# dkaslovsky/GraphRole

Measured on AMD Instinct MI355X. Metric: ReFeX edges-aggregated/sec (+ RolX NMF iters/sec in nmf.iters_per_s), 1M-node graph, higher is better.
Workload: dtype f64; 1 GPU; ba1m; description=Barabasi-Albert n=1,000,000 m=10 (~10M edges), seed 0  [BASELINE config 3/4], n_nodes=1000000, n_edges=9999900, nnz=19999800, n_roles=6, n_features=20

## Files before the change

### graphrole_amd/csrc/grx_common.h

```cpp
#pragma once
#include <hip/hip_runtime.h>

#include <cstdint>
#include <cstdio>

#include "grx.h"

void grx_set_error(const char *fmt, ...);

#define GRX_CHECK_HIP(expr)                                                                   \
    do {                                                                                      \
        hipError_t e__ = (expr);                                                              \
        if (e__ != hipSuccess) {                                                              \
            grx_set_error("%s:%d: %s -> %s", __FILE__, __LINE__, #expr, hipGetErrorString(e__)); \
            return GRX_ERR_HIP;                                                               \
        }                                                                                     \
    } while (0)

#define GRX_REQUIRE(cond, ...)                                                                \
    do {                                                                                      \
        if (!(cond)) {                                                                        \
            grx_set_error(__VA_ARGS__);                                                       \
            return GRX_ERR_INVALID;                                                           \
        }                                                                                     \
// ... 37 lines not shown
static inline size_t grx_align_up(size_t x, size_t a) { return (x + a - 1) / a * a; }

static inline unsigned grx_grid(int64_t items, int64_t per_block, int64_t cap)
{
    const int64_t g = grx_ceil_div(items, per_block);
    return (unsigned)(g < 1 ? 1 : g > cap ? cap : g);
}

void grx_fill32(int32_t *d_dst, int64_t count, int32_t value, hipStream_t st);
void grx_fill64(uint64_t *d_dst, int64_t count, uint64_t value, hipStream_t st);

struct SpPull {
    int64_t n;
    const int64_t *row_ptr;
    const int32_t *col;
    const double *w;
    const int32_t *hub_rows;
    int64_t n_hub_rows, hub_degree;
};

enum { GRX_CT_DONE = 0, GRX_CT_LEVEL, GRX_CT_FOUND, GRX_CT_BFS_WORDS };
constexpr int GRX_CTRL_MAX_WORDS = 16;

int grx_read_ctrl(const int32_t *d_ctrl, int words, int32_t *out, hipStream_t st);

int grx_frontier_advance(int32_t *d_ctrl, hipStream_t st);

template <class Enqueue>
int grx_run_rounds(const char *what, int batch, int64_t max_rounds, int words, const int32_t *d_ctrl, int32_t *h,
                   hipStream_t st, Enqueue enqueue_one)
{
    for (int k = 0; k < words; ++k) h[k] = 0;
    int64_t issued = 0;
    while (!h[0]) {
        GRX_REQUIRE(issued <= max_rounds, what, (long long)issued);
        for (int k = 0; k < batch; ++k, ++issued) {
            const int rc = enqueue_one();
            if (rc != GRX_OK) return rc;
            GRX_LAUNCH_CHECK();
        }
        const int rc = grx_read_ctrl(d_ctrl, words, h, st);
        if (rc != GRX_OK) return rc;
    }
    return GRX_OK;
}

int grx_internal_sort_columns(int64_t n, int ncols, const double *cols, int64_t ld, double *out, int64_t out_ld,
                              void *workspace, hipStream_t st);
int grx_internal_sort_pairs(int64_t n, const double *col, double *out, uint32_t *perm, void *workspace, hipStream_t st);
size_t grx_internal_sort_pairs_workspace_bytes(int64_t n);
int grx_internal_sort_u64(int64_t n, const uint64_t *keys, uint64_t *out, void *workspace, hipStream_t st);
int grx_internal_vertical_log_bin(int64_t n, int ncols, const double *d_cols, int64_t ld, const uint8_t *h_is_i64, double frac,
                                  uint8_t *d_bins, int64_t ld_bins, int32_t *d_nbins, void *d_workspace,
                                  size_t workspace_bytes, int32_t *d_status, void *stream);
int64_t grx_internal_plan_max_degree(const grx_aggregate_plan *plan);

#ifndef GRX_NT_STREAMS
#define GRX_NT_STREAMS 0
#endif
#if GRX_NT_STREAMS
#define GRX_STREAM_LD(p) __builtin_nontemporal_load(&(p))
#define GRX_STREAM_ST(p, v) __builtin_nontemporal_store((v), &(p))
#else
#define GRX_STREAM_LD(p) (p)
#define GRX_STREAM_ST(p, v) ((p) = (v))
#endif

template <int WIDTH>
__device__ __forceinline__ double grx_group_sum(double v)
{
#pragma unroll
    for (int off = WIDTH / 2; off > 0; off >>= 1) v += __shfl_xor(v, off, WIDTH);
    return v;
}

template <int WIDTH>
__device__ __forceinline__ double grx_group_max(double v)
{
#pragma unroll
    for (int off = WIDTH / 2; off > 0; off >>= 1) v = fmax(v, __shfl_xor(v, off, WIDTH));
    return v;
}

template <int BLOCK, bool MAX = false>
__device__ __forceinline__ double grx_block_reduce(double v, double *sm)
{
    const int t = threadIdx.x;
    sm[t] = v;
    __syncthreads();
#pragma unroll
    for (int s = BLOCK / 2; s > 0; s >>= 1) {
        if (t < s) sm[t] = MAX ? fmax(sm[t], sm[t + s]) : sm[t] + sm[t + s];
        __syncthreads();
    }
    const double r = sm[0];
    __syncthreads();
    return r;
}
```

### graphrole_amd/csrc/grx_prune.hip

```cpp
#include "grx_sort.h"

#include <cstdlib>

namespace {

struct BinPlanCol {
    uint64_t const_bits;
    uint8_t narrow;
    uint8_t npass;
    uint8_t lo_shift;
    uint8_t pad0;
    uint8_t dshift[4];
};

struct ColFlags { uint64_t w[8]; };
constexpr int MAX_TYPED_COLS = 512;
__device__ __forceinline__ bool col_is_i64(const ColFlags &f, int col) { return col < MAX_TYPED_COLS && ((f.w[col >> 6] >> (col & 63)) & 1ull); }
__device__ __forceinline__ uint64_t i64_bits_to_key(double raw) { return (uint64_t)__double_as_longlong(raw) ^ 0x8000000000000000ull; }
__device__ __forceinline__ uint64_t value_key(double raw, bool is_i64) { return is_i64 ? i64_bits_to_key(raw) : f64_to_key(raw + 0.0); }

constexpr int BITS_TILE = 256 * 32;
constexpr int LO_SHIFT_INT = 255;

__global__ __launch_bounds__(256) void key_bits_kernel(const double *__restrict__ cols, int64_t ld, int64_t n,
// ... 688 lines not shown
                pq[u] = act[u] ? pair_pq[id] : 0u;
            }
            uint2 x[U], y[U];
#pragma unroll
            for (int u = 0; u < U; ++u) {
                act[u] = act[u] && (int)cur[u] <= cap;
                x[u] = *reinterpret_cast<const uint2 *>(tile + (pq[u] >> 8) * CH_STRIDE + lane * 8);
                y[u] = *reinterpret_cast<const uint2 *>(tile + (pq[u] & 0xFF) * CH_STRIDE + lane * 8);
            }
#pragma unroll
            for (int u = 0; u < U; ++u) {
                if (!act[u]) continue;
                const int id = id0 + 4 * u;
                uint32_t m = ch_absdiff_max4(x[u].x, y[u].x);
                const uint32_t m2 = ch_absdiff_max4(x[u].y, y[u].y);
                m = m2 > m ? m2 : m;
                if (__ballot((int)m > cap) != 0) {
                    if (lane == 0) pair_max[id] = (uint8_t)(cap + 1);
                    continue;
                }
#pragma unroll
                for (int off = 32; off > 0; off >>= 1) {
                    const uint32_t o = __shfl_xor(m, off, 64);
                    m = o > m ? o : m;
                }
                if (lane == 0 && m > cur[u]) pair_max[id] = (uint8_t)m;
            }
        }
    }
    __syncthreads();
    for (int id = threadIdx.x; id < npairs; id += 256) {
        const int mx = pair_max[id];
        if (mx == 0) continue;
        const int lp = pair_pq[id] >> 8, lq = pair_pq[id] & 0xFF;
        const int p = lp < na ? a0 + lp : b0 + (lp - na), q = lq < na ? a0 + lq : b0 + (lq - na);
        if (__hip_atomic_load(&dist[(size_t)p * ldF + q], __ATOMIC_RELAXED, __HIP_MEMORY_SCOPE_AGENT) < mx) {
            atomicMax(&dist[(size_t)p * ldF + q], mx);
            atomicMax(&dist[(size_t)q * ldF + p], mx);
        }
    }
}

constexpr int SEL_NB = 4096;
constexpr int SEL_MAX_IDS = 512;
constexpr int SEL_SORT_CAP = 8192;
constexpr uint16_t SEL_MARK_SORTED = 0x8000;
constexpr uint16_t SEL_MARK_TIES = 0xFFFF;
constexpr uint16_t SEL_THR_EXACT = 0x8000;
inline int64_t sel_bid_min_n()
{
    static const int64_t v = [] { const char *e = std::getenv("GRX_BIN_BID_MIN_N"); return e ? (int64_t)std::atoll(e) : (int64_t)2500000; }();
    return v;
}
__host__ __device__ inline int64_t sel_bid_stride(int64_t n) { return (n + 3) & ~(int64_t)3; }
constexpr int SEL_HIST_ITEMS = 32;
constexpr int SEL_HIST_TILE = 256 * SEL_HIST_ITEMS;
struct SelMap { uint64_t kmin; int shift; int ncells; int nb; };
constexpr int SEL_NSAMPLE = SEL_NB - 1;

__device__ __forceinline__ int sel_bucket(const SelMap &m, const uint32_t *__restrict__ lut, uint64_t key)
{
    if (key <= m.kmin) return 0;
    const uint64_t rel = key - m.kmin;
    uint64_t c = rel >> m.shift;
    if (c >= (uint64_t)m.ncells) return m.nb - 1;
    const uint32_t e = lut[c];
    const int k = (int)(e >> 16);
    const uint64_t within = rel - (c << m.shift);
    return (int)(e & 0xFFFFu) + (int)(within >> (m.shift - k));
}

constexpr int SEL_MAX_TIES = 511;

__global__ __launch_bounds__(1024) void sel_map_kernel(const double *__restrict__ cols, int64_t ld, int64_t n,
                                                       SelMap *__restrict__ maps, uint32_t *__restrict__ luts,
                                                       uint16_t *__restrict__ tie_of_bucket, uint64_t *__restrict__ tie_value,
                                                       uint32_t *__restrict__ hist, uint32_t *__restrict__ cursor,
                                                       unsigned long long *__restrict__ bmin,
                                                       unsigned long long *__restrict__ bmax, uint8_t *__restrict__ tie_broken,
                                                       int32_t *__restrict__ fault, ColFlags flags)
{
    for (int b = threadIdx.x; b < SEL_NB; b += 1024) {
        const size_t cell = (size_t)blockIdx.x * SEL_NB + b;
        hist[cell] = 0; cursor[cell] = 0; bmax[cell] = 0ull; bmin[cell] = ~0ull; tie_broken[cell] = 0;
    }
    if (blockIdx.x == 0 && threadIdx.x == 0) *fault = 0;
    __shared__ unsigned long long smin[SEL_NB];
    __shared__ unsigned long long smax[SEL_NB];
    __shared__ uint32_t scnt[SEL_NB];
    __shared__ uint32_t s_lut[SEL_NB];
    __shared__ uint32_t cnt[SEL_NB];
    __shared__ uint64_t red[32];
    __shared__ uint32_t wsum[16];
    __shared__ SelMap s_map;
    const int col = blockIdx.x, t = threadIdx.x, lane = t & 63, wave = t >> 6;
    const bool i64 = col_is_i64(flags, col);
    const double *x = cols + (size_t)col * ld;
    uint64_t key[4];
    bool have[4];
    uint64_t mn = ~0ull, mx = 0ull;
#pragma unroll
    for (int j = 0; j < 4; ++j) {
        const int64_t k = (int64_t)t * 4 + j;
        have[j] = k < SEL_NSAMPLE && (n > SEL_NSAMPLE || k < n);
        key[j] = 0;
        if (have[j]) {
            key[j] = value_key(x[n > SEL_NSAMPLE ? (k * (n - 1)) / (SEL_NSAMPLE - 1) : k], i64);
            mn = key[j] < mn ? key[j] : mn;
            mx = key[j] > mx ? key[j] : mx;
        }
        cnt[4 * t + j] = 0;
    }
#pragma unroll
    for (int off = 32; off > 0; off >>= 1) {
        const uint64_t a = __shfl_xor(mn, off, 64), b = __shfl_xor(mx, off, 64);
        mn = a < mn ? a : mn;
        mx = b > mx ? b : mx;
    }
    if (lane == 0) { red[wave] = mn; red[16 + wave] = mx; }
    __syncthreads();
    if (t == 0) {
        for (int w = 1; w < 16; ++w) { mn = red[w] < mn ? red[w] : mn; mx = red[16 + w] > mx ? red[16 + w] : mx; }
        const uint64_t span = mx - mn;
        const int bits = span ? 64 - __clzll((long long)span) : 0;
        s_map.kmin = mn;
        s_map.shift = bits > 12 ? bits - 12 : 0;
        s_map.ncells = (int)(span >> s_map.shift) + 1;
        s_map.nb = 0;
    }
    __syncthreads();
    const SelMap m = s_map;
#pragma unroll
    for (int j = 0; j < 4; ++j)
// ... 19 lines not shown
    __syncthreads();
    uint32_t run = inc - local;
    for (int w = 0; w < wave; ++w) run += wsum[w];
    uint32_t *lut = luts + (size_t)col * SEL_NB;
#pragma unroll
    for (int j = 0; j < 4; ++j) {
        const uint32_t e = run | (kk[j] << 16);
        lut[4 * t + j] = e;
        s_lut[4 * t + j] = e;
        run += alloc[j];
        smin[4 * t + j] = ~0ull; smax[4 * t + j] = 0ull; scnt[4 * t + j] = 0;
    }
    if (t == 1023) {
        s_map.nb = (int)run + 1;
        maps[col] = s_map;
    }
    __syncthreads();
    const SelMap mm = s_map;
#pragma unroll
    for (int j = 0; j < 4; ++j) {
        if (have[j]) {
            const int b = sel_bucket(mm, s_lut, key[j]);
            atomicAdd(&scnt[b], 1u);
            atomicMin(&smin[b], (unsigned long long)key[j]);
            atomicMax(&smax[b], (unsigned long long)key[j]);
        }
    }
    __syncthreads();
    uint32_t cand[4];
#pragma unroll
    for (int j = 0; j < 4; ++j) { const int b = 4 * t + j; cand[j] = (scnt[b] >= 2 && smin[b] == smax[b]) ? 1u : 0u; }
    const uint32_t lc = cand[0] + cand[1] + cand[2] + cand[3];
    uint32_t ic = lc;
#pragma unroll
    for (int off = 1; off < 64; off <<= 1) {
        const uint32_t y = __shfl_up(ic, off, 64);
        if (lane >= off) ic += y;
    }
    __syncthreads();
    if (lane == 63) wsum[wave] = ic;
    __syncthreads();
    uint32_t id = ic - lc;
    for (int w = 0; w < wave; ++w) id += wsum[w];
#pragma unroll
    for (int j = 0; j < 4; ++j) {
        const int b = 4 * t + j;
        uint16_t tid = 0;
        if (cand[j]) {
            ++id;
            if (id <= SEL_MAX_TIES) { tid = (uint16_t)id; tie_value[(size_t)col * (SEL_MAX_TIES + 1) + id] = smin[b]; }
        }
        tie_of_bucket[(size_t)col * SEL_NB + b] = tid;
    }
}

template <bool STORE_BID>
__global__ __launch_bounds__(256) void sel_hist_kernel(const double *__restrict__ cols, int64_t ld, int64_t n,
                                                       const SelMap *__restrict__ maps, const uint32_t *__restrict__ luts,
                                                       const uint16_t *__restrict__ tie_of_bucket,
                                                       const uint64_t *__restrict__ tie_value, uint8_t *__restrict__ tie_broken,
                                                       uint32_t *__restrict__ hist, uint16_t *__restrict__ bid, ColFlags flags,
                                                       int tiles_per_wg)
{
    __shared__ uint32_t h[SEL_NB];
    __shared__ uint32_t lut[SEL_NB];
    __shared__ uint16_t tieb[SEL_NB];
    __shared__ uint64_t tiev[SEL_MAX_TIES + 1];
    const int col = blockIdx.y;
    const bool i64 = col_is_i64(flags, col);
    const SelMap m = maps[col];
    for (int b = threadIdx.x; b < SEL_NB; b += 256) {
        h[b] = 0;
        lut[b] = luts[(size_t)col * SEL_NB + b];
        tieb[b] = tie_of_bucket[(size_t)col * SEL_NB + b];
    }
    for (int k = threadIdx.x; k <= SEL_MAX_TIES; k += 256) tiev[k] = tie_value[(size_t)col * (SEL_MAX_TIES + 1) + k];
    __syncthreads();
    const double *x = cols + (size_t)col * ld;
    const int64_t last = n - 1;
    const int lane = threadIdx.x & 63;
    for (int tile = 0; tile < tiles_per_wg; ++tile) {
    const int64_t base = ((int64_t)blockIdx.x * tiles_per_wg + tile) * SEL_HIST_TILE;
    if (base >= n) break;
    for (int i0 = 0; i0 < SEL_HIST_ITEMS; i0 += 8) {
        double raw[8];
#pragma unroll
        for (int j = 0; j < 8; ++j) {
            const int64_t idx = base + (int64_t)(i0 + j) * 256 + threadIdx.x;
            raw[j] = x[idx < n ? idx : last];
        }
        __builtin_amdgcn_sched_barrier(0);
#pragma unroll
        for (int j = 0; j < 8; ++j) {
            const bool valid = base + (int64_t)(i0 + j) * 256 + threadIdx.x < n;
            const uint64_t key = value_key(raw[j], i64);
            const int b = sel_bucket(m, lut, key);
            if (STORE_BID && valid)
                bid[(size_t)col * sel_bid_stride(n) + base + (int64_t)(i0 + j) * 256 + threadIdx.x] = (uint16_t)b;
            const int tid = valid ? (int)tieb[b] : 0;
            if (tid && tiev[tid] != key) tie_broken[(size_t)col * SEL_NB + b] = 1;
            const uint64_t active = __ballot(valid);
            if (active == 0) continue;
            const int b0 = __shfl(b, __ffsll((long long)active) - 1, 64);
            if (__ballot(valid && b != b0) == 0) {
                if (lane == __ffsll((long long)active) - 1) atomicAdd(&h[b0], (uint32_t)__popcll(active));
            } else if (valid) {
                atomicAdd(&h[b], 1u);
            }
        }
    }
    }
    __syncthreads();
    uint32_t *out = hist + (size_t)col * SEL_NB;
    for (int b = threadIdx.x; b < SEL_NB; b += 256)
        if (h[b]) atomicAdd(&out[b], h[b]);
}

__global__ __launch_bounds__(1024) void sel_walk1_kernel(int64_t n, double frac,
                                                         const uint32_t *__restrict__ hist, const uint16_t *__restrict__ tie_of_bucket,
                                                         const uint8_t *__restrict__ tie_broken,
                                                         const uint64_t *__restrict__ tie_value, uint32_t *__restrict__ cum,
                                                         uint16_t *__restrict__ mark, uint32_t *__restrict__ seg_off,
                                                         uint16_t *__restrict__ idlist, int32_t *__restrict__ nids,
                                                         unsigned long long *__restrict__ bmin,
                                                         unsigned long long *__restrict__ bmax)
{
    __shared__ uint8_t TIE[SEL_NB];
    __shared__ uint32_t C[SEL_NB];
    __shared__ uint32_t S[SEL_NB];
    __shared__ uint8_t M[SEL_NB];
    __shared__ uint32_t wsum[16];
    const int col = blockIdx.x, t = threadIdx.x, lane = t & 63, wave = t >> 6;
    constexpr int nb = SEL_NB;
    const uint32_t *h = hist + (size_t)col * SEL_NB;
    auto scan4 = [&](uint32_t (&v)[4], uint32_t *dst) {
        const uint32_t local = v[0] + v[1] + v[2] + v[3];
        uint32_t inc = local;
#pragma unroll
        for (int off = 1; off < 64; off <<= 1) {
            const uint32_t y = __shfl_up(inc, off, 64);
            if (lane >= off) inc += y;
        }
        __syncthreads();
        if (lane == 63) wsum[wave] = inc;
        __syncthreads();
        uint32_t before = inc - local;
        for (int w = 0; w < wave; ++w) before += wsum[w];
        uint32_t run = before;
#pragma unroll
        for (int j = 0; j < 4; ++j) { run += v[j]; dst[4 * t + j] = run; }
        __syncthreads();
    };
    uint32_t v[4];
#pragma unroll
    for (int j = 0; j < 4; ++j) {
        const int b = 4 * t + j;
        v[j] = b < nb ? h[b] : 0u;
        M[b] = 0;
        TIE[b] = (tie_of_bucket[(size_t)col * SEL_NB + b] != 0 && tie_broken[(size_t)col * SEL_NB + b] == 0) ? 1 : 0;
    }
    scan4(v, C);
    if (wave == 0) {
        auto bucket_of = [&](int64_t pos) {
            const int coarse = lane * 64 + 63;
            const bool gt = coarse < nb ? (int64_t)C[coarse] > pos : true;
            const int blk = __ffsll((long long)__ballot(gt)) - 1;
            const int fine = blk * 64 + lane;
            const bool gt2 = fine < nb ? (int64_t)C[fine] > pos : true;
            return blk * 64 + __ffsll((long long)__ballot(gt2)) - 1;
        };
        int64_t dlo = 0, dhi = 0;
        for (int step = 0; step < GRX_MAX_BINS && dlo < n; ++step) {
            int64_t slo = (int64_t)(frac * (double)(n - dlo));
            if (slo < 1) slo = 1;
            const int64_t plo = dlo + slo - 1;
            const int64_t dh = dhi < n ? dhi : n - 1;
            int64_t shi = (int64_t)(frac * (double)(n - dh));
            if (shi < 1) shi = 1;
            int64_t phi = dh + shi - 1;
            if (phi < plo) phi = plo;
            const int jlo = bucket_of(plo), jhi = bucket_of(phi);
            for (int j = jlo + lane; j <= jhi; j += 64) M[j] = 1;
            dlo = TIE[jlo] ? (int64_t)C[jlo] : plo + 1;
            dhi = (int64_t)C[jhi];
            if (dhi < dlo) dhi = dlo;
        }
    }
    __syncthreads();
    bool collect[4];
#pragma unroll
    for (int j = 0; j < 4; ++j) {
        const int b = 4 * t + j;
        const uint32_t cnt = b < nb ? (C[b] - (b ? C[b - 1] : 0u)) : 0u;
        collect[j] = M[b] && !TIE[b];
        v[j] = collect[j] ? cnt : 0u;
        if (M[b] && TIE[b]) {
            const size_t cell = (size_t)col * SEL_NB + b;
            const uint64_t value = tie_value[(size_t)col * (SEL_MAX_TIES + 1) + tie_of_bucket[cell]];
            bmin[cell] = value;
            bmax[cell] = value;
        }
    }
    scan4(v, S);
#pragma unroll
    for (int j = 0; j < 4; ++j) {
        const int b = 4 * t + j;
        if (b < nb) {
            cum[(size_t)col * SEL_NB + b] = C[b];
            seg_off[(size_t)col * SEL_NB + b] = S[b] - v[j];
        }
    }
    uint32_t m[4];
#pragma unroll
    for (int j = 0; j < 4; ++j) m[j] = collect[j] ? 1u : 0u;
    scan4(m, S);
#pragma unroll
    for (int j = 0; j < 4; ++j) {
        const int b = 4 * t + j;
        if (b < nb) {
            const uint32_t id = S[b];
            uint16_t mk = 0;
            if (m[j]) {
                mk = (uint16_t)(id < SEL_MAX_IDS ? id : SEL_MAX_IDS);
                if (id < SEL_MAX_IDS) idlist[(size_t)col * SEL_MAX_IDS + id - 1] = (uint16_t)b;
            } else if (M[b]) {
                mk = SEL_MARK_TIES;
            }
            mark[(size_t)col * SEL_NB + b] = mk;
        }
    }
    if (t == 1023) nids[col] = (int32_t)(S[nb - 1] < (uint32_t)SEL_MAX_IDS ? S[nb - 1] : SEL_MAX_IDS - 1);
}

__global__ __launch_bounds__(512) void sel_sort_kernel(const uint32_t *__restrict__ cum, const uint32_t *__restrict__ seg_off,
                                                       const uint16_t *__restrict__ idlist, const int32_t *__restrict__ nids,
                                                       const unsigned long long *__restrict__ bmin,
                                                       const unsigned long long *__restrict__ bmax, int64_t n,
                                                       uint64_t *__restrict__ coll, uint16_t *__restrict__ mark)
{
    __shared__ uint64_t s[SEL_SORT_CAP];
    const int col = blockIdx.y;
    const int count = nids[col];
    for (int id = blockIdx.x; id < count; id += gridDim.x) {
        const int b = idlist[(size_t)col * SEL_MAX_IDS + id];
        const size_t cell = (size_t)col * SEL_NB + b;
        const int64_t len = (int64_t)cum[cell] - (b ? (int64_t)cum[cell - 1] : 0);
        if (len < 2 || len > SEL_SORT_CAP || bmin[cell] == bmax[cell]) continue;
        uint64_t *seg = coll + (size_t)col * n + seg_off[cell];
        int P = 2;
        while (P < len) P <<= 1;
        __syncthreads();
        for (int i = threadIdx.x; i < P; i += 512) s[i] = i < len ? seg[i] : ~0ull;
        for (int k = 2; k <= P; k <<= 1) {
            for (int j = k >> 1; j > 0; j >>= 1) {
                __syncthreads();
                for (int i = threadIdx.x; i < P / 2; i += 512) {
                    const int lo = 2 * i - (i & (j - 1)), hi = lo + j;
                    const uint64_t a = s[lo], c = s[hi];
                    const bool up = (lo & k) == 0;
                    if ((a > c) == up) { s[lo] = c; s[hi] = a; }
                }
            }
        }
        __syncthreads();
        for (int i = threadIdx.x; i < len; i += 512) seg[i] = s[i];
        if (threadIdx.x == 0) mark[cell] |= SEL_MARK_SORTED;
    }
}

template <bool FROM_BID>
__global__ __launch_bounds__(256) void sel_collect_kernel(const double *__restrict__ cols, int64_t ld, int64_t n,
                                                          const uint16_t *__restrict__ bid,
                                                          const SelMap *__restrict__ maps, const uint32_t *__restrict__ luts,
                                                          const uint16_t *__restrict__ mark,
                                                          const uint32_t *__restrict__ seg_off, uint32_t *__restrict__ cursor,
                                                          uint64_t *__restrict__ coll, unsigned long long *__restrict__ bmin,
                                                          unsigned long long *__restrict__ bmax, ColFlags flags,
                                                          int tiles_per_wg)
{
    __shared__ uint32_t cnt[SEL_MAX_IDS];
    __shared__ uint32_t basev[SEL_MAX_IDS];
    __shared__ uint16_t bucket_of_id[SEL_MAX_IDS];
    __shared__ unsigned long long lo_id[SEL_MAX_IDS];
    __shared__ unsigned long long hi_id[SEL_MAX_IDS];
    __shared__ uint16_t M[SEL_NB];
    __shared__ uint32_t lut[SEL_NB];
    const int col = blockIdx.y;
    const bool i64 = col_is_i64(flags, col);
    const SelMap m = maps[col];
    for (int b = threadIdx.x; b < SEL_NB; b += 256) { M[b] = mark[(size_t)col * SEL_NB + b]; lut[b] = FROM_BID ? 0u : luts[(size_t)col * SEL_NB + b]; }
    const double *x = cols + (size_t)col * ld;
    const int64_t last = n - 1;
    for (int tile = 0; tile < tiles_per_wg; ++tile) {
    const int64_t base = ((int64_t)blockIdx.x * tiles_per_wg + tile) * SORT_TILE;
    if (base >= n) break;
    __syncthreads();
    for (int k = threadIdx.x; k < SEL_MAX_IDS; k += 256) { cnt[k] = 0; lo_id[k] = ~0ull; hi_id[k] = 0ull; }
    __syncthreads();
    double raw[SORT_ITEMS];
    uint16_t bv[SORT_ITEMS];
    const uint16_t *bx = FROM_BID ? bid + (size_t)col * sel_bid_stride(n) : nullptr;
#pragma unroll
    for (int i = 0; i < SORT_ITEMS; ++i) {
// ... 288 lines not shown
{
    SelLayout L;
    size_t o = 0;
    auto take = [&](size_t bytes) { const size_t at = o; o += grx_align_up(bytes, 256); return at; };
    L.maps = take((size_t)ncols * sizeof(SelMap));
    L.luts = take((size_t)ncols * SEL_NB * 4);
    L.tieb = take((size_t)ncols * SEL_NB * 2);
    L.tiev = take((size_t)ncols * (SEL_MAX_TIES + 1) * 8);
    L.hist = take((size_t)ncols * SEL_NB * 4);
    L.cursor = take((size_t)ncols * SEL_NB * 4);
    L.bmax = take((size_t)ncols * SEL_NB * 8);
    L.tbroken = take((size_t)ncols * SEL_NB);
    L.bmin = take((size_t)ncols * SEL_NB * 8);
    L.cum = take((size_t)ncols * SEL_NB * 4);
    L.seg_off = take((size_t)ncols * SEL_NB * 4);
    L.mark = take((size_t)ncols * SEL_NB * 2);
    L.idlist = take((size_t)ncols * SEL_MAX_IDS * 2);
    L.nids = take((size_t)ncols * 4);
    L.coll = take((size_t)ncols * (size_t)n * 8);
    L.bid = take(n >= sel_bid_min_n() ? (size_t)ncols * (size_t)sel_bid_stride(n) * 2 : 0);
    L.thr = take((size_t)ncols * GRX_MAX_BINS * 8);
    L.thrb = take((size_t)ncols * GRX_MAX_BINS * 2);
    L.nbins = take((size_t)ncols * 4);
    L.fault = take(4);
    L.total = o;
    return L;
}
}

size_t grx_log_bin_workspace_bytes(int64_t n, int ncols)
{
    if (n <= 0 || ncols <= 0) return 256;
    const SortPlan p = make_plan(n, ncols);
    const size_t sort_path = 2 * p.keys_bytes + p.hist_bytes + grx_align_up((size_t)ncols * GRX_MAX_BINS * 8, 256) +
                             grx_align_up((size_t)ncols * 4, 256) + grx_align_up((size_t)ncols * p.ntiles * 32, 256) +
                             grx_align_up((size_t)ncols * sizeof(BinPlanCol), 256);
    const size_t select_path = sel_layout(n, ncols).total;
    return sort_path > select_path ? sort_path : select_path;
}

int grx_vertical_log_bin(int64_t n, int ncols, const double *d_cols, int64_t ld, double frac,
                         uint8_t *d_bins, int64_t ld_bins, int32_t *d_nbins, void *d_workspace,
                         size_t workspace_bytes, void *stream)
{
    return grx_vertical_log_bin_typed(n, ncols, d_cols, ld, nullptr, frac, d_bins, ld_bins, d_nbins, d_workspace,
                                      workspace_bytes, stream);
}

int grx_vertical_log_bin_typed(int64_t n, int ncols, const double *d_cols, int64_t ld, const uint8_t *h_is_i64, double frac,
                               uint8_t *d_bins, int64_t ld_bins, int32_t *d_nbins, void *d_workspace,
                               size_t workspace_bytes, void *stream)
{
    return grx_internal_vertical_log_bin(n, ncols, d_cols, ld, h_is_i64, frac, d_bins, ld_bins, d_nbins, d_workspace,
                                         workspace_bytes, nullptr, stream);
}

}

int grx_internal_vertical_log_bin(int64_t n, int ncols, const double *d_cols, int64_t ld, const uint8_t *h_is_i64, double frac,
                                  uint8_t *d_bins, int64_t ld_bins, int32_t *d_nbins, void *d_workspace,
                                  size_t workspace_bytes, int32_t *status, void *stream)
{
    ColFlags flags;
    for (int j = 0; j < 8; ++j) flags.w[j] = 0;
    if (h_is_i64)
        for (int c = 0; c < ncols; ++c)
            if (h_is_i64[c]) {
                GRX_REQUIRE(c < MAX_TYPED_COLS, "grx_vertical_log_bin_typed: int64 columns beyond the first %d of a call", MAX_TYPED_COLS);
                flags.w[c >> 6] |= 1ull << (c & 63);
            }
    GRX_REQUIRE(frac > 0.0 && frac < 1.0, "must specify frac in interval (0, 1)");
    GRX_REQUIRE(n >= 0 && ncols >= 0 && ld >= n && ld_bins >= n, "grx_vertical_log_bin: bad shape");
    GRX_REQUIRE(n < ((int64_t)1 << 31), "grx_vertical_log_bin: n must be < 2^31");
    if (n == 0 || ncols == 0) return GRX_OK;
    GRX_REQUIRE(d_cols && d_bins && d_workspace, "grx_vertical_log_bin: NULL pointer");
    if (workspace_bytes < grx_log_bin_workspace_bytes(n, ncols)) {
        grx_set_error("grx_vertical_log_bin: workspace %zu < %zu", workspace_bytes, grx_log_bin_workspace_bytes(n, ncols));
        return GRX_ERR_WORKSPACE;
    }
    hipStream_t st = grx_stream(stream);
    const SortPlan p = make_plan(n, ncols);
    char *ws = reinterpret_cast<char *>(d_workspace);
    static const bool use_sort = [] { const char *e = std::getenv("GRX_BIN_SORT"); return e && *e == '1'; }();
    if (!use_sort) {
        const SelLayout L = sel_layout(n, ncols);
        SelMap *maps = reinterpret_cast<SelMap *>(ws + L.maps);
        uint32_t *luts = reinterpret_cast<uint32_t *>(ws + L.luts);
        uint16_t *tieb = reinterpret_cast<uint16_t *>(ws + L.tieb);
        uint64_t *tiev = reinterpret_cast<uint64_t *>(ws + L.tiev);
        uint8_t *tbroken = reinterpret_cast<uint8_t *>(ws + L.tbroken);
        uint32_t *hist = reinterpret_cast<uint32_t *>(ws + L.hist);
        uint32_t *cursor = reinterpret_cast<uint32_t *>(ws + L.cursor);
        uint32_t *cum = reinterpret_cast<uint32_t *>(ws + L.cum);
        uint32_t *seg_off = reinterpret_cast<uint32_t *>(ws + L.seg_off);
        uint16_t *mark = reinterpret_cast<uint16_t *>(ws + L.mark);
        uint16_t *idlist = reinterpret_cast<uint16_t *>(ws + L.idlist);
        int32_t *nids = reinterpret_cast<int32_t *>(ws + L.nids);
        uint64_t *coll = reinterpret_cast<uint64_t *>(ws + L.coll);
        uint64_t *thr = reinterpret_cast<uint64_t *>(ws + L.thr);
        uint16_t *bid = reinterpret_cast<uint16_t *>(ws + L.bid);
        uint16_t *thrb = reinterpret_cast<uint16_t *>(ws + L.thrb);
        const bool use_bid = n >= sel_bid_min_n();
        int32_t *nb_ws = reinterpret_cast<int32_t *>(ws + L.nbins);
        int32_t *fault = reinterpret_cast<int32_t *>(ws + L.fault);
        unsigned long long *bmin = reinterpret_cast<unsigned long long *>(ws + L.bmin);
        unsigned long long *bmax = reinterpret_cast<unsigned long long *>(ws + L.bmax);
        {
            GRX_PROF(GRX_K_SEL_MAP, st);
            sel_map_kernel<<<ncols, 1024, 0, st>>>(d_cols, ld, n, maps, luts, tieb, tiev, hist, cursor, bmin, bmax, tbroken, fault, flags);
        }
        {
            GRX_PROF(GRX_K_SEL_HIST, st);
            const int hist_tiles = use_bid ? 4 : 1;
            const dim3 hgrid((unsigned)grx_ceil_div(n, (int64_t)SEL_HIST_TILE * hist_tiles), ncols);
            if (use_bid) sel_hist_kernel<true><<<hgrid, 256, 0, st>>>(d_cols, ld, n, maps, luts, tieb, tiev, tbroken, hist, bid, flags, hist_tiles);
            else sel_hist_kernel<false><<<hgrid, 256, 0, st>>>(d_cols, ld, n, maps, luts, tieb, tiev, tbroken, hist, nullptr, flags, hist_tiles);
        }
        {
            GRX_PROF(GRX_K_SEL_WALK1, st);
            sel_walk1_kernel<<<ncols, 1024, 0, st>>>(n, frac, hist, tieb, tbroken, tiev, cum, mark, seg_off, idlist, nids, bmin, bmax);
        }
        {
            GRX_PROF(GRX_K_SEL_COLLECT, st);
            const int coll_tiles = use_bid ? 8 : 1;
            const dim3 cgrid((unsigned)grx_ceil_div(p.ntiles, coll_tiles), ncols);
            if (use_bid) sel_collect_kernel<true><<<cgrid, 256, 0, st>>>(d_cols, ld, n, bid, maps, luts, mark, seg_off, cursor, coll, bmin, bmax, flags, coll_tiles);
            else sel_collect_kernel<false><<<cgrid, 256, 0, st>>>(d_cols, ld, n, nullptr, maps, luts, mark, seg_off, cursor, coll, bmin, bmax, flags, coll_tiles);
        }
        {
            GRX_PROF(GRX_K_SEL_SEGSORT, st);
            sel_sort_kernel<<<dim3(64, ncols), 512, 0, st>>>(cum, seg_off, idlist, nids, bmin, bmax, n, coll, mark);
        }
        {
            GRX_PROF(GRX_K_SEL_WALK2, st);
            sel_walk2_kernel<<<ncols, 256, 0, st>>>(n, frac, cum, mark, seg_off, coll, bmin, bmax, thr, use_bid ? thrb : nullptr, nb_ws, fault);
        }
        GRX_LAUNCH_CHECK();
        const int64_t want = grx_ceil_div(n, 256 * 4);
        const dim3 grid((unsigned)(want > 2048 ? 2048 : want), ncols);
        {
            GRX_PROF(GRX_K_BIN_ASSIGN, st);
            const int64_t want_a = grx_ceil_div(n, 256 * 4 * 16);
            const dim3 agrid((unsigned)(want_a > 2048 ? 2048 : want_a), ncols);
            if (use_bid) sel_assign_kernel<<<agrid, 256, 0, st>>>(d_cols, ld, n, bid, thr, thrb, nb_ws, d_bins, ld_bins, flags, fault, status);
            else bin_assign_kernel<<<grid, 256, 0, st>>>(d_cols, ld, n, thr, nb_ws, d_bins, ld_bins, flags, fault, status);
        }
        GRX_LAUNCH_CHECK();
        if (d_nbins)
            GRX_CHECK_HIP(hipMemcpyAsync(d_nbins, nb_ws, (size_t)ncols * 4, hipMemcpyDeviceToDevice, st));
        return GRX_OK;
    }
    uint64_t *buf_a = reinterpret_cast<uint64_t *>(ws);
    uint64_t *buf_b = reinterpret_cast<uint64_t *>(ws + p.keys_bytes);
    uint32_t *hist = reinterpret_cast<uint32_t *>(ws + 2 * p.keys_bytes);
    uint32_t *tot = hist + grx_align_up((size_t)ncols * RADIX * (size_t)p.ntiles * 4, 256) / 4;
    uint64_t *thr = reinterpret_cast<uint64_t *>(ws + 2 * p.keys_bytes + p.hist_bytes);
    int32_t *nb_ws = reinterpret_cast<int32_t *>(ws + 2 * p.keys_bytes + p.hist_bytes +
                                                 grx_align_up((size_t)ncols * GRX_MAX_BINS * 8, 256));
    char *plan_ws = reinterpret_cast<char *>(nb_ws) + grx_align_up((size_t)ncols * 4, 256);
    uint64_t *bits = reinterpret_cast<uint64_t *>(plan_ws);
    BinPlanCol *plan = reinterpret_cast<BinPlanCol *>(plan_ws + grx_align_up((size_t)ncols * p.ntiles * 32, 256));
    const int nbt = (int)grx_ceil_div(n, BITS_TILE);
    {
        GRX_PROF(GRX_K_KEY_BITS, st);
        key_bits_kernel<<<dim3(nbt, ncols), 256, 0, st>>>(d_cols, ld, n, nbt, bits, flags);
        bin_plan_kernel<<<ncols, 64, 0, st>>>(bits, nbt, plan);
    }
    GRX_LAUNCH_CHECK();
    const dim3 sgrid(p.ntiles, ncols);
    for (int round = 0; round < 4; ++round) {
        {
            GRX_PROF(GRX_K_SORT_COUNT, st);
            tile_count2_kernel<<<sgrid, SORT_THREADS, 0, st>>>(d_cols, ld, n, round, p.ntiles, plan, buf_a, buf_b, hist, flags);
        }
        {
            GRX_PROF(GRX_K_SORT_SCAN, st);
            scan_rows2_kernel<<<dim3(RADIX, ncols), 64, 0, st>>>(hist, p.ntiles, tot, plan, round);
        }
        {
            GRX_PROF(GRX_K_SORT_SCATTER, st);
            scatter2_kernel<<<sgrid, SORT_THREADS, 0, st>>>(d_cols, ld, n, round, p.ntiles, plan, buf_a, buf_b, hist, tot, flags);
        }
        GRX_LAUNCH_CHECK();
    }
// ... 80 lines not shown
```

### graphrole_amd/csrc/grx_refex.hip

```cpp
#include "grx_common.h"

#include <algorithm>
#include <cstdlib>
#include <cstring>
#include <string>
#include <vector>

namespace {

const char *const AGG_NAMES[] = {"sum", "mean", "min", "max", "var", "std", "prod", "median", "count", "size"};
constexpr int N_AGG_KINDS = 10;

struct Column {
    std::string name;
    int generation;
    int parent;
    int agg;
    const double *data;
    const uint8_t *bins;
    int record_index;
    bool int32_exact = false;
    int kind = 0;
    int base = -1;
    int bits = -1;
// ... 143 lines not shown
                  int f0, const double *const *h_gen0_cols, const char *const *h_gen0_names, const int *h_gen0_int32,
                  int max_generations, int n_aggs, const int *h_aggs, grx_comm *comm, const int64_t *h_bounds, void *d_arena,
                  size_t arena_bytes, grx_grow_fn grow, void *grow_user, int max_columns,
                  grx_refex_column *h_columns, int *n_columns, int max_gens, grx_refex_generation *h_gens,
                  int *generation_count, size_t *arena_needed, void *stream)
{
    GRX_REQUIRE(plan && d_row_ptr && d_agg_col && n >= 1 && f0 >= 1 && h_gen0_cols && h_gen0_names,
                "grx_refex_run: bad graph / generation-0 arguments");
    GRX_REQUIRE(n_aggs >= 1 && h_aggs && h_columns && n_columns && h_gens && generation_count && max_columns >= f0 &&
                max_gens >= 1, "grx_refex_run: bad output arguments");
    bool has[N_AGG_KINDS] = {};
    for (int a = 0; a < n_aggs; ++a) {
        GRX_REQUIRE(h_aggs[a] >= 0 && h_aggs[a] < N_AGG_KINDS, "grx_refex_run: unknown aggregation id %d", h_aggs[a]);
        has[h_aggs[a]] = true;
    }
    hipStream_t st = grx_stream(stream);
    const int P = comm ? grx_comm_world(comm) : 1, me = comm ? grx_comm_rank(comm) : 0;
    GRX_REQUIRE(!comm || h_bounds, "grx_refex_run: a communicator needs the row partition h_bounds");
    if (comm)
        GRX_REQUIRE(h_bounds[0] == 0 && h_bounds[P] == n, "grx_refex_run: h_bounds must run from 0 to n");
    const int64_t rb = comm ? h_bounds[me] : 0, re = comm ? h_bounds[me + 1] : n;
    Arena arena(d_arena, d_arena ? arena_bytes : 0, grow, grow_user);
    int64_t nnz_rows = 0;
    if (has[GRX_AGG_MEDIAN]) {
        std::vector<int64_t> ends(P + 1, 0);
        for (int q = 0; q <= P; ++q)
            GRX_CHECK_HIP(hipMemcpyAsync(&ends[q], d_row_ptr + (comm ? h_bounds[q] : (q ? n : 0)), 8, hipMemcpyDeviceToHost, st));
        GRX_CHECK_HIP(hipStreamSynchronize(st));
        for (int q = 0; q < P; ++q) nnz_rows = std::max(nnz_rows, ends[q + 1] - ends[q]);
    }
    std::vector<Column> cols;
    std::vector<int> work;
    std::vector<std::vector<int>> recorded;
    int n_out = 0;
    bool table_full = false;

    int deg_bits = 1;
    while (deg_bits < 62 && (grx_internal_plan_max_degree(plan) >> deg_bits) != 0) ++deg_bits;
    static const bool packed_allowed = [] { const char *e = std::getenv("GRX_NO_PACKED_ROWS"); return !(e && *e == '1'); }();
    int gather_row_bytes = 0;
    auto update = [&](int first_new, int count, const double *block, int generation, bool partial) -> int {
        const size_t scratch_mark = arena.top;
        uint8_t *bins = nullptr;
        if (count) {
            arena.rewind(scratch_mark);
            bins = reinterpret_cast<uint8_t *>(arena.take((size_t)count * n));
        }
        const size_t persistent_top = arena.top;
        const int n_owned = comm ? (count > me ? (count - me + P - 1) / P : 0) : count;
        const int n_owned_max = comm ? (count + P - 1) / P : count;
        const int bin_batch = grx_refex_bin_batch(n, n_owned_max);
        const size_t ws_bytes = grx_log_bin_workspace_bytes(n, bin_batch);
        void *ws = n_owned_max ? arena.take(ws_bytes) : nullptr;
        auto bin_columns = [&](int ncols, const double *src_cols, int64_t ld_cols, uint8_t *dst_bins, int32_t *d_status) -> int {
            for (int c0 = 0; c0 < ncols; c0 += bin_batch) {
                const int b = ncols - c0 < bin_batch ? ncols - c0 : bin_batch;
                GRX_TRY(grx_internal_vertical_log_bin(n, b, src_cols + (size_t)c0 * ld_cols, ld_cols, nullptr, 0.5,
                                                      dst_bins + (size_t)c0 * n, n, nullptr, ws, ws_bytes, d_status, stream));
            }
            return GRX_OK;
        };
        double *owned = (comm && partial && n_owned_max) ? reinterpret_cast<double *>(arena.take((size_t)n_owned_max * n * 8)) : nullptr;
        uint8_t *owned_bins = (comm && n_owned_max) ? reinterpret_cast<uint8_t *>(arena.take((size_t)n_owned_max * n)) : nullptr;
        for (int j = 0; j < count; ++j) work.push_back(first_new + j);
        const int F = (int)work.size();
        const bool want_bits = count <= 64 && generation + 1 < max_generations && packed_allowed;
        const size_t tail_words = 2 + (size_t)(want_bits ? count : 0);
        const size_t dist_bytes = grx_align_up(((size_t)F * F + tail_words) * 4, 256);
        int32_t *d_dist = reinterpret_cast<int32_t *>(arena.take(dist_bytes));
        std::vector<int> drop_idx;
        if (!arena.overflow) {
            if (F >= 2) GRX_CHECK_HIP(hipMemsetAsync(d_dist, 0, dist_bytes, st));
            if (count && !comm) {
                GRX_TRY(bin_columns(count, block, n, bins, F >= 2 ? d_dist + (size_t)F * F : nullptr));
            } else if (count) {
                const double *src = block + (size_t)me * n;
                int64_t ld_src = (int64_t)P * n;
                if (partial) {
                    GRX_TRY(grx_comm_columns_to_owners(comm, h_bounds, count, block, n, 8, owned, n, stream));
                    src = owned;
                    ld_src = n;
                }
                if (n_owned) {
                    GRX_TRY(bin_columns(n_owned, src, ld_src, owned_bins, F >= 2 ? d_dist + (size_t)F * F : nullptr));
                }
                GRX_TRY(grx_comm_owned_to_rows(comm, h_bounds, count, owned_bins, n, 1, bins, n, stream));
            }
            for (int j = 0; j < count; ++j) cols[first_new + j].bins = bins + (size_t)j * n;
            if (F >= 2 && tail_words > 2 && re > rb) {
                uint64_t mask = 0;
                for (int j = 0; j < count; ++j)
                    if (cols[first_new + j].kind == 1) mask |= 1ull << j;
                if (mask) GRX_TRY(grx_column_bits(n, count, block, n, rb, re, mask, d_dist + (size_t)F * F + 2, stream));
            }
            if (F >= 2) {
                std::vector<const uint8_t *> ptrs(F);
                for (int j = 0; j < F; ++j) ptrs[j] = cols[work[j]].bins;
                if (re > rb) GRX_TRY(grx_chebyshev(rb, re, F, 0, ptrs.data(), d_dist, generation, stream));
                if (comm) GRX_TRY(grx_comm_all_reduce(comm, d_dist, (size_t)F * F + tail_words, GRX_I32, GRX_MAX, stream));
                void *host = nullptr;
                GRX_TRY(pinned(((size_t)F * F + tail_words) * 4, &host));
                GRX_TRY(grx_fetch_begin(host, d_dist, ((size_t)F * F + tail_words) * 4, st));
                GRX_TRY(grx_fetch_wait(st));
                if (tail_words > 2)
                    for (int j = 0; j < count; ++j) {
                        const int32_t b = reinterpret_cast<const int32_t *>(host)[(size_t)F * F + 2 + j];
                        if (cols[first_new + j].kind == 1 && b >= 1 && b <= 62) cols[first_new + j].bits = b;
                    }
                const int32_t walk_failed = reinterpret_cast<const int32_t *>(host)[(size_t)F * F];
                const int32_t bins_overflow = reinterpret_cast<const int32_t *>(host)[(size_t)F * F + 1];
                if (walk_failed != 0 || bins_overflow != 0) {
                    grx_set_error("grx_refex_run: generation %d: vertical log binning failed on some rank (%s%s); "
                                  "GRX_BIN_SORT=1 selects the sort-based binning", generation,
                                  walk_failed ? "the sort-free threshold walk met an unmarked bucket" : "",
                                  bins_overflow ? " a column needs more than GRX_MAX_BINS bins" : "");
                    return GRX_ERR_UNSUPPORTED;
                }
                drop_idx = prune(cols, work, reinterpret_cast<const int32_t *>(host), generation, recorded);
            }
        }
        arena.rewind(persistent_top);
        std::vector<char> dropped(cols.size(), 0);
        for (int m : drop_idx) dropped[work[m]] = 1;
        const int working_before = F;
        work.erase(std::remove_if(work.begin(), work.end(), [&](int c) { return dropped[c] != 0; }), work.end());
        std::vector<int> kept;
        for (int j = 0; j < count; ++j)
            if (!dropped[first_new + j]) kept.push_back(first_new + j);
        if (comm && partial && !kept.empty() && !arena.overflow) {
            std::vector<void *> ptrs;
            for (int c : kept) ptrs.push_back(const_cast<double *>(cols[c].data));
            GRX_TRY(grx_comm_all_gather_rows(comm, h_bounds, (int)ptrs.size(), ptrs.data(), 8, stream));
        }
        if (!drop_idx.empty())
            std::stable_sort(kept.begin(), kept.end(), [&](int a, int b) { return cols[a].name < cols[b].name; });
        for (int c : kept) {
            if (n_out >= max_columns) { table_full = true; break; }
// ... 164 lines not shown
```

Baseline: 16.06 billion edges/s.

## Fuse dist-buffer clear into binning map kernel, register-resident segment sort, single-pass walk scan

Result: slower. 15.61 billion edges/s (-2.8%).

```diff
diff --git a/graphrole_amd/csrc/grx_common.h b/graphrole_amd/csrc/grx_common.h
--- a/graphrole_amd/csrc/grx_common.h
+++ b/graphrole_amd/csrc/grx_common.h
@@ -113,7 +113,7 @@
 int grx_internal_sort_u64(int64_t n, const uint64_t *keys, uint64_t *out, void *workspace, hipStream_t st);
 int grx_internal_vertical_log_bin(int64_t n, int ncols, const double *d_cols, int64_t ld, const uint8_t *h_is_i64, double frac,
                                   uint8_t *d_bins, int64_t ld_bins, int32_t *d_nbins, void *d_workspace,
-                                  size_t workspace_bytes, int32_t *d_status, void *stream);
+                                  size_t workspace_bytes, int32_t *d_status, void *d_clear, size_t clear_bytes, void *stream);
 int64_t grx_internal_plan_max_degree(const grx_aggregate_plan *plan);
 
 #ifndef GRX_NT_STREAMS
diff --git a/graphrole_amd/csrc/grx_prune.hip b/graphrole_amd/csrc/grx_prune.hip
--- a/graphrole_amd/csrc/grx_prune.hip
+++ b/graphrole_amd/csrc/grx_prune.hip
@@ -764,6 +764,16 @@
     static const int64_t v = [] { const char *e = std::getenv("GRX_BIN_BID_MIN_N"); return e ? (int64_t)std::atoll(e) : (int64_t)2500000; }();
     return v;
 }
+constexpr int SEL_REG_SORT_CAP = 2048;
+inline int sel_reg_sort_cap()
+{
+    static const int v = [] {
+        const char *e = std::getenv("GRX_BIN_REG_SORT_CAP");
+        const long long c = e ? std::atoll(e) : (long long)SEL_REG_SORT_CAP;
+        return (int)(c < 0 ? 0 : (c > SEL_REG_SORT_CAP ? SEL_REG_SORT_CAP : c));
+    }();
+    return v;
+}
 __host__ __device__ inline int64_t sel_bid_stride(int64_t n) { return (n + 3) & ~(int64_t)3; }
 constexpr int SEL_HIST_ITEMS = 32;
 constexpr int SEL_HIST_TILE = 256 * SEL_HIST_ITEMS;
@@ -790,7 +800,8 @@
                                                        uint32_t *__restrict__ hist, uint32_t *__restrict__ cursor,
                                                        unsigned long long *__restrict__ bmin,
                                                        unsigned long long *__restrict__ bmax, uint8_t *__restrict__ tie_broken,
-                                                       int32_t *__restrict__ fault, ColFlags flags)
+                                                       int32_t *__restrict__ fault, ColFlags flags,
+                                                       uint32_t *__restrict__ clear_words, size_t n_clear_words)
 {
     for (int b = threadIdx.x; b < SEL_NB; b += 1024) {
         const size_t cell = (size_t)blockIdx.x * SEL_NB + b;
@@ -916,6 +927,7 @@
         }
         tie_of_bucket[(size_t)col * SEL_NB + b] = tid;
     }
+    for (size_t i = (size_t)blockIdx.x * 1024 + threadIdx.x; i < n_clear_words; i += (size_t)gridDim.x * 1024) clear_words[i] = 0u;
 }
 
 template <bool STORE_BID>
@@ -991,39 +1003,47 @@
 {
     __shared__ uint8_t TIE[SEL_NB];
     __shared__ uint32_t C[SEL_NB];
-    __shared__ uint32_t S[SEL_NB];
     __shared__ uint8_t M[SEL_NB];
-    __shared__ uint32_t wsum[16];
+    __shared__ unsigned long long wsum[16];
     const int col = blockIdx.x, t = threadIdx.x, lane = t & 63, wave = t >> 6;
     constexpr int nb = SEL_NB;
     const uint32_t *h = hist + (size_t)col * SEL_NB;
-    auto scan4 = [&](uint32_t (&v)[4], uint32_t *dst) {
-        const uint32_t local = v[0] + v[1] + v[2] + v[3];
-        uint32_t inc = local;
+    auto before_me = [&](unsigned long long local) {
+        unsigned long long inc = local;
 #pragma unroll
         for (int off = 1; off < 64; off <<= 1) {
-            const uint32_t y = __shfl_up(inc, off, 64);
+            const unsigned long long y = __shfl_up(inc, off, 64);
             if (lane >= off) inc += y;
         }
         __syncthreads();
         if (lane == 63) wsum[wave] = inc;
         __syncthreads();
-        uint32_t before = inc - local;
-        for (int w = 0; w < wave; ++w) before += wsum[w];
-        uint32_t run = before;
-#pragma unroll
-        for (int j = 0; j < 4; ++j) { run += v[j]; dst[4 * t + j] = run; }
-        __syncthreads();
+        unsigned long long ws = wsum[lane & 15];
+#pragma unroll
+        for (int off = 1; off < 16; off <<= 1) {
+            const unsigned long long y = __shfl_up(ws, off, 16);
+            if ((lane & 15) >= off) ws += y;
+        }
+        const unsigned long long earlier = __shfl(ws, wave ? wave - 1 : 0, 64);
+        return inc - local + (wave ? earlier : 0ull);
     };
-    uint32_t v[4];
+    const uint4 h4 = *reinterpret_cast<const uint4 *>(h + 4 * t);
+    const uint2 tob4 = *reinterpret_cast<const uint2 *>(tie_of_bucket + (size_t)col * SEL_NB + 4 * t);
+    const uint32_t broken4 = *reinterpret_cast<const uint32_t *>(tie_broken + (size_t)col * SEL_NB + 4 * t);
+    uint32_t v[4] = {h4.x, h4.y, h4.z, h4.w};
+    const uint16_t tob[4] = {(uint16_t)tob4.x, (uint16_t)(tob4.x >> 16), (uint16_t)tob4.y, (uint16_t)(tob4.y >> 16)};
 #pragma unroll
     for (int j = 0; j < 4; ++j) {
         const int b = 4 * t + j;
-        v[j] = b < nb ? h[b] : 0u;
         M[b] = 0;
-        TIE[b] = (tie_of_bucket[(size_t)col * SEL_NB + b] != 0 && tie_broken[(size_t)col * SEL_NB + b] == 0) ? 1 : 0;
-    }
-    scan4(v, C);
+        TIE[b] = (tob[j] != 0 && ((broken4 >> (8 * j)) & 0xFFu) == 0) ? 1 : 0;
+    }
+    {
+        uint32_t run = (uint32_t)before_me((unsigned long long)v[0] + v[1] + v[2] + v[3]);
+#pragma unroll
+        for (int j = 0; j < 4; ++j) { run += v[j]; C[4 * t + j] = run; }
+        __syncthreads();
+    }
     if (wave == 0) {
         auto bucket_of = [&](int64_t pos) {
             const int coarse = lane * 64 + 63;
@@ -1051,68 +1071,96 @@
         }
     }
     __syncthreads();
-    bool collect[4];
+    bool collect[4], marked[4];
+    uint64_t value[4];
+    uint32_t m = 0;
 #pragma unroll
     for (int j = 0; j < 4; ++j) {
         const int b = 4 * t + j;
-        const uint32_t cnt = b < nb ? (C[b] - (b ? C[b - 1] : 0u)) : 0u;
-        collect[j] = M[b] && !TIE[b];
-        v[j] = collect[j] ? cnt : 0u;
-        if (M[b] && TIE[b]) {
-            const size_t cell = (size_t)col * SEL_NB + b;
-            const uint64_t value = tie_value[(size_t)col * (SEL_MAX_TIES + 1) + tie_of_bucket[cell]];
-            bmin[cell] = value;
-            bmax[cell] = value;
-        }
-    }
-    scan4(v, S);
+        marked[j] = M[b] != 0;
+        collect[j] = marked[j] && !TIE[b];
+        m += collect[j] ? 1u : 0u;
+        value[j] = (marked[j] && !collect[j]) ? tie_value[(size_t)col * (SEL_MAX_TIES + 1) + tob[j]] : 0ull;
+        if (!collect[j]) v[j] = 0u;
+    }
+    const unsigned long long front = before_me((unsigned long long)(v[0] + v[1] + v[2] + v[3]) | ((unsigned long long)m << 32));
+    uint32_t off = (uint32_t)front, id = (uint32_t)(front >> 32);
 #pragma unroll
     for (int j = 0; j < 4; ++j) {
         const int b = 4 * t + j;
-        if (b < nb) {
-            cum[(size_t)col * SEL_NB + b] = C[b];
-            seg_off[(size_t)col * SEL_NB + b] = S[b] - v[j];
-        }
-    }
-    uint32_t m[4];
-#pragma unroll
-    for (int j = 0; j < 4; ++j) m[j] = collect[j] ? 1u : 0u;
-    scan4(m, S);
-#pragma unroll
-    for (int j = 0; j < 4; ++j) {
-        const int b = 4 * t + j;
-        if (b < nb) {
-            const uint32_t id = S[b];
-            uint16_t mk = 0;
-            if (m[j]) {
-                mk = (uint16_t)(id < SEL_MAX_IDS ? id : SEL_MAX_IDS);
-                if (id < SEL_MAX_IDS) idlist[(size_t)col * SEL_MAX_IDS + id - 1] = (uint16_t)b;
-            } else if (M[b]) {
-                mk = SEL_MARK_TIES;
-            }
-            mark[(size_t)col * SEL_NB + b] = mk;
-        }
-    }
-    if (t == 1023) nids[col] = (int32_t)(S[nb - 1] < (uint32_t)SEL_MAX_IDS ? S[nb - 1] : SEL_MAX_IDS - 1);
+        cum[(size_t)col * SEL_NB + b] = C[b];
+        seg_off[(size_t)col * SEL_NB + b] = off;
+        off += v[j];
+        uint16_t mk = 0;
+        if (collect[j]) {
+            ++id;
+            mk = (uint16_t)(id < SEL_MAX_IDS ? id : SEL_MAX_IDS);
+            if (id < SEL_MAX_IDS) idlist[(size_t)col * SEL_MAX_IDS + id - 1] = (uint16_t)b;
+        } else if (marked[j]) {
+            mk = SEL_MARK_TIES;
+            bmin[(size_t)col * SEL_NB + b] = value[j];
+            bmax[(size_t)col * SEL_NB + b] = value[j];
+        }
+        mark[(size_t)col * SEL_NB + b] = mk;
+    }
+    if (t == 1023) nids[col] = (int32_t)(id < (uint32_t)SEL_MAX_IDS ? id : SEL_MAX_IDS - 1);
 }
 
 __global__ __launch_bounds__(512) void sel_sort_kernel(const uint32_t *__restrict__ cum, const uint32_t *__restrict__ seg_off,
                                                        const uint16_t *__restrict__ idlist, const int32_t *__restrict__ nids,
                                                        const unsigned long long *__restrict__ bmin,
                                                        const unsigned long long *__restrict__ bmax, int64_t n,
-                                                       uint64_t *__restrict__ coll, uint16_t *__restrict__ mark)
+                                                       uint64_t *__restrict__ coll, uint16_t *__restrict__ mark, int reg_cap)
 {
     __shared__ uint64_t s[SEL_SORT_CAP];
     const int col = blockIdx.y;
     const int count = nids[col];
+    const int b_first = idlist[(size_t)col * SEL_MAX_IDS + blockIdx.x];
     for (int id = blockIdx.x; id < count; id += gridDim.x) {
-        const int b = idlist[(size_t)col * SEL_MAX_IDS + id];
+        const int b = id == (int)blockIdx.x ? b_first : (int)idlist[(size_t)col * SEL_MAX_IDS + id];
         const size_t cell = (size_t)col * SEL_NB + b;
         const int64_t len = (int64_t)cum[cell] - (b ? (int64_t)cum[cell - 1] : 0);
         if (len < 2 || len > SEL_SORT_CAP || bmin[cell] == bmax[cell]) continue;
         uint64_t *seg = coll + (size_t)col * n + seg_off[cell];
         int P = 2;
         while (P < len) P <<= 1;
+        if (len <= reg_cap) {
+            const int t = threadIdx.x, e0 = 4 * t;
+            uint64_t x[4];
+#pragma unroll
+            for (int r = 0; r < 4; ++r) x[r] = e0 + r < (int)len ? seg[e0 + r] : ~0ull;
+            auto keep = [](uint64_t mine, uint64_t other, bool smaller) { return (other < mine) == smaller ? other : mine; };
+            for (int k = 2; k <= P; k <<= 1) {
+                for (int j = k >> 1; j > 0; j >>= 1) {
+                    uint64_t y[4];
+                    if (j >= 256) {
+                        __syncthreads();
+#pragma unroll
+                        for (int r = 0; r < 4; ++r) s[e0 + r] = x[r];
+                        __syncthreads();
+#pragma unroll
+                        for (int r = 0; r < 4; ++r) y[r] = s[(e0 ^ j) + r];
+                    } else if (j >= 4) {
+#pragma unroll
+                        for (int r = 0; r < 4; ++r) y[r] = __shfl_xor((unsigned long long)x[r], j >> 2, 64);
+                    } else if (j == 2) {
+                        y[0] = x[2]; y[1] = x[3]; y[2] = x[0]; y[3] = x[1];
+                    } else {
+                        y[0] = x[1]; y[1] = x[0]; y[2] = x[3]; y[3] = x[2];
+                    }
+#pragma unroll
+                    for (int r = 0; r < 4; ++r) {
+                        const int e = e0 + r;
+                        x[r] = keep(x[r], y[r], ((e & k) == 0) == ((e & j) == 0));
+                    }
+                }
+            }
+#pragma unroll
+            for (int r = 0; r < 4; ++r)
+                if (e0 + r < (int)len) seg[e0 + r] = x[r];
+            if (threadIdx.x == 0) mark[cell] |= SEL_MARK_SORTED;
+            continue;
+        }
         __syncthreads();
         for (int i = threadIdx.x; i < P; i += 512) s[i] = i < len ? seg[i] : ~0ull;
         for (int k = 2; k <= P; k <<= 1) {
@@ -1507,14 +1555,14 @@
                                size_t workspace_bytes, void *stream)
 {
     return grx_internal_vertical_log_bin(n, ncols, d_cols, ld, h_is_i64, frac, d_bins, ld_bins, d_nbins, d_workspace,
-                                         workspace_bytes, nullptr, stream);
+                                         workspace_bytes, nullptr, nullptr, 0, stream);
 }
 
 }
 
 int grx_internal_vertical_log_bin(int64_t n, int ncols, const double *d_cols, int64_t ld, const uint8_t *h_is_i64, double frac,
                                   uint8_t *d_bins, int64_t ld_bins, int32_t *d_nbins, void *d_workspace,
-                                  size_t workspace_bytes, int32_t *status, void *stream)
+                                  size_t workspace_bytes, int32_t *status, void *d_clear, size_t clear_bytes, void *stream)
 {
     ColFlags flags;
     for (int j = 0; j < 8; ++j) flags.w[j] = 0;
@@ -1527,6 +1575,10 @@
     GRX_REQUIRE(frac > 0.0 && frac < 1.0, "must specify frac in interval (0, 1)");
     GRX_REQUIRE(n >= 0 && ncols >= 0 && ld >= n && ld_bins >= n, "grx_vertical_log_bin: bad shape");
     GRX_REQUIRE(n < ((int64_t)1 << 31), "grx_vertical_log_bin: n must be < 2^31");
+    GRX_REQUIRE(clear_bytes % 4 == 0 && (d_clear || clear_bytes == 0), "grx_vertical_log_bin: bad buffer to clear");
+    static const bool use_sort = [] { const char *e = std::getenv("GRX_BIN_SORT"); return e && *e == '1'; }();
+    if (clear_bytes && (n == 0 || ncols == 0 || use_sort))
+        GRX_CHECK_HIP(hipMemsetAsync(d_clear, 0, clear_bytes, grx_stream(stream)));
     if (n == 0 || ncols == 0) return GRX_OK;
     GRX_REQUIRE(d_cols && d_bins && d_workspace, "grx_vertical_log_bin: NULL pointer");
     if (workspace_bytes < grx_log_bin_workspace_bytes(n, ncols)) {
@@ -1536,7 +1588,6 @@
     hipStream_t st = grx_stream(stream);
     const SortPlan p = make_plan(n, ncols);
     char *ws = reinterpret_cast<char *>(d_workspace);
-    static const bool use_sort = [] { const char *e = std::getenv("GRX_BIN_SORT"); return e && *e == '1'; }();
     if (!use_sort) {
         const SelLayout L = sel_layout(n, ncols);
         SelMap *maps = reinterpret_cast<SelMap *>(ws + L.maps);
@@ -1562,7 +1613,8 @@
         unsigned long long *bmax = reinterpret_cast<unsigned long long *>(ws + L.bmax);
         {
             GRX_PROF(GRX_K_SEL_MAP, st);
-            sel_map_kernel<<<ncols, 1024, 0, st>>>(d_cols, ld, n, maps, luts, tieb, tiev, hist, cursor, bmin, bmax, tbroken, fault, flags);
+            sel_map_kernel<<<ncols, 1024, 0, st>>>(d_cols, ld, n, maps, luts, tieb, tiev, hist, cursor, bmin, bmax, tbroken, fault, flags,
+                                                   reinterpret_cast<uint32_t *>(d_clear), clear_bytes / 4);
         }
         {
             GRX_PROF(GRX_K_SEL_HIST, st);
@@ -1584,7 +1636,7 @@
         }
         {
             GRX_PROF(GRX_K_SEL_SEGSORT, st);
-            sel_sort_kernel<<<dim3(64, ncols), 512, 0, st>>>(cum, seg_off, idlist, nids, bmin, bmax, n, coll, mark);
+            sel_sort_kernel<<<dim3(64, ncols), 512, 0, st>>>(cum, seg_off, idlist, nids, bmin, bmax, n, coll, mark, sel_reg_sort_cap());
         }
         {
             GRX_PROF(GRX_K_SEL_WALK2, st);
diff --git a/graphrole_amd/csrc/grx_refex.hip b/graphrole_amd/csrc/grx_refex.hip
--- a/graphrole_amd/csrc/grx_refex.hip
+++ b/graphrole_amd/csrc/grx_refex.hip
@@ -219,11 +219,13 @@
         const int bin_batch = grx_refex_bin_batch(n, n_owned_max);
         const size_t ws_bytes = grx_log_bin_workspace_bytes(n, bin_batch);
         void *ws = n_owned_max ? arena.take(ws_bytes) : nullptr;
-        auto bin_columns = [&](int ncols, const double *src_cols, int64_t ld_cols, uint8_t *dst_bins, int32_t *d_status) -> int {
+        auto bin_columns = [&](int ncols, const double *src_cols, int64_t ld_cols, uint8_t *dst_bins, int32_t *d_status,
+                               void *d_clear, size_t clear_bytes) -> int {
             for (int c0 = 0; c0 < ncols; c0 += bin_batch) {
                 const int b = ncols - c0 < bin_batch ? ncols - c0 : bin_batch;
                 GRX_TRY(grx_internal_vertical_log_bin(n, b, src_cols + (size_t)c0 * ld_cols, ld_cols, nullptr, 0.5,
-                                                      dst_bins + (size_t)c0 * n, n, nullptr, ws, ws_bytes, d_status, stream));
+                                                      dst_bins + (size_t)c0 * n, n, nullptr, ws, ws_bytes, d_status,
+                                                      c0 == 0 ? d_clear : nullptr, c0 == 0 ? clear_bytes : 0, stream));
             }
             return GRX_OK;
         };
@@ -237,9 +239,11 @@
         int32_t *d_dist = reinterpret_cast<int32_t *>(arena.take(dist_bytes));
         std::vector<int> drop_idx;
         if (!arena.overflow) {
-            if (F >= 2) GRX_CHECK_HIP(hipMemsetAsync(d_dist, 0, dist_bytes, st));
+            const bool clear_in_binning = count && !comm && F >= 2;
+            if (F >= 2 && !clear_in_binning) GRX_CHECK_HIP(hipMemsetAsync(d_dist, 0, dist_bytes, st));
             if (count && !comm) {
-                GRX_TRY(bin_columns(count, block, n, bins, F >= 2 ? d_dist + (size_t)F * F : nullptr));
+                GRX_TRY(bin_columns(count, block, n, bins, F >= 2 ? d_dist + (size_t)F * F : nullptr,
+                                    clear_in_binning ? d_dist : nullptr, clear_in_binning ? dist_bytes : 0));
             } else if (count) {
                 const double *src = block + (size_t)me * n;
                 int64_t ld_src = (int64_t)P * n;
@@ -249,7 +253,7 @@
                     ld_src = n;
                 }
                 if (n_owned) {
-                    GRX_TRY(bin_columns(n_owned, src, ld_src, owned_bins, F >= 2 ? d_dist + (size_t)F * F : nullptr));
+                    GRX_TRY(bin_columns(n_owned, src, ld_src, owned_bins, F >= 2 ? d_dist + (size_t)F * F : nullptr, nullptr, 0));
                 }
                 GRX_TRY(grx_comm_owned_to_rows(comm, h_bounds, count, owned_bins, n, 1, bins, n, stream));
             }
```
